# neuromodulation/py_neuromodulation

Hardware: AMD Instinct MI355X
Metric: windows/sec (all features), 256 ch @ 1 kHz (higher is better)
Workload: dtype f32; 1 GPU; 256ch/GPU @1kHz, W=1000, hop=100, 1024 hops/step, all 9 hot-path features, 4 bands, notch50+CAR, z-score normalisation; channels_per_gpu=256, features_per_window=9984, parallelism=channel-shard x1, no collective

## Files before the change

py_neuromodulation_amd/csrc/nmx_engine.inc:

```

#include <algorithm>
#include <chrono>
#include <cmath>
#include <cstdio>
#include <cstdlib>
#include <cstring>
#include <map>
#include <string>
#include <thread>
#include <deque>
#include <functional>
#include <mutex>
#include <condition_variable>
#include <pthread.h>
#include <vector>

#include "../../include/nmx.h"
#include "nmx_k_coh.h"
#include "nmx_k_proj.h"

static thread_local std::string g_nmx_err;
static int nmx_fail(int code, const std::string& msg) {
  g_nmx_err = msg;
  return code;
// ... 44 lines not shown
  NmxFirKernel kernel = NMX_FIR_ONE;
  bool pipelined = false;
  const float* hc = nullptr;
  const float* twc = nullptr;
  bool fused = false;
};
struct FirStage {
  NmxBankArgs a{};
  bool w64 = false;
  NmxBankW64Args w{};
  std::vector<FirLaunch> launches;
  bool takes_dc = true;
};

struct BurstStage {
  NmxHilbertArgs hil{};
  NmxBurstThrArgs bthr{};
  NmxBurstStatArgs bstat{};
  NmxHilbertKind hil_kind = NMX_HIL_FIXED128;
  bool own_hilbert = false;
  bool sparse = false;
  bool sparse_count = false;
  long long env_tail_rows = 0, env_rows = 0;
  NmxBurstStatKind stat_kind = NMX_BSTAT_GENERIC;
  NmxBurstWalk walk{};
  bool fill_split = true;
  int nt_thr = 256;
  long long seen = 0;
  float* d_top = nullptr;
  long long* d_counts = nullptr;
  size_t top_bytes = 0, counts_bytes = 0;
  float* d_floor = nullptr;
  Buf env[2], thr[2];
  Buf env_full[2];
  Buf yb;
  Buf slots;
  int fill_hops(int nw) const { return walk.fill && seen == 0 ? nmx_burst_fill_hops(bthr, nw) : 0; }
};
struct SharpStage {
  NmxSharpArgs a{};
  NmxSharpKind kind = NMX_SHARP_LIST;
  Buf swy[2], todo[2];
  Buf slab;
};
struct KalmanStage {
  NmxKalmanArgs a{};
  double* d_state = nullptr;
  size_t bytes = 0;
};
struct RawNormStage {
  NmxRawNormArgs a{};
  long long hops = 0;
  bool sorted_valid = false;
  size_t ring_bytes = 0, cnt_bytes = 0, len_bytes = 0;
  Buf x_rn, mean, scale;
  Buf qt, qn;
};
// ... 134 lines not shown
```

py_neuromodulation_amd/csrc/nmx_engine_plan_bursts.inc:

```

int build_hilbert(Plan& P) {
  const nmx_plan_desc& d = P.d;
  NmxHilbertArgs& H = P.bursts.hil;
  H.W = d.window;
  H.hil_full = d.window & 1;
  int rc;
  if ((rc = build_fft(P, H.hil_full ? d.window : d.window / 2, &H.hil_r, true))) return rc;
  if ((rc = build_fft(P, d.window, &H.hil_c, true))) return rc;
  H.off_a = 0;
  if (H.hil_full) {
    H.off_b = al4(2 * d.window);
    H.off_y = H.off_b;
    H.lds_floats = H.off_b + al4(2 * d.window);
  } else {
    H.off_b = al4(d.window + 2);
    H.off_y = H.off_b + al4(d.window + 2);
    H.lds_floats = H.off_y + al4(d.window);
  }
  NMX_REQUIRE(H.lds_floats * 4 <= 160 * 1024, "window too long for the Hilbert kernel");
  H.w500_tab = nullptr;
  H.w1000_tab = nullptr;
  if (d.window == 1000) {
    if ((rc = build_w500_tab(P))) return rc;
    H.w500_tab = P.w500_tab;
// ... 6 lines not shown
      t[2 * i + 1] = (float)(scale * std::sin(ang));
    };
    for (int lane = 0; lane < 64; ++lane) {
      const int l = lane < 50 ? lane : 0, k = l % 10;
      for (int r = 1; r < 10; ++r) {
        put((r - 1) * 64 + lane, -2.0 * kPi * ((10 * k * r) % 1000) / 1000.0, 1.0);
        put((8 + r) * 64 + lane, -2.0 * kPi * ((l * r) % 1000) / 1000.0, 1.0);
        put((17 + r) * 64 + lane, -2.0 * kPi * (((l + 50) * r) % 1000) / 1000.0, 1.0);
      }
    }
    for (int k = 0; k < NMX_W1000_CS_N; ++k) put(NMX_W1000_TW_N + k, 2.0 * kPi * k / 2000.0, k ? 2.0 / 2000.0 : 0.0);
    H.w1000_tab = (const float*)upload(P, t.data(), t.size() * sizeof(float));
    if (!H.w1000_tab) return nmx_fail(NMX_E_NOMEM, "table allocation failed");
  }
#endif
  const bool wave = env_int("NMX_HILBERT_W500", 1) != 0;
  P.bursts.hil_kind = wave && d.window == 1000 ? NMX_HIL_W500 : wave && H.w1000_tab ? NMX_HIL_W1000 : NMX_HIL_FIXED128;
  return 0;
}

void burst_floor_reset(Plan& P) {
  const std::vector<float> f((size_t)P.d.n_channels * P.d.n_burst_bands, -INFINITY);
  be_h2d_sync(P.bursts.d_floor, f.data(), f.size() * sizeof(float));
}

static size_t burst_state_bytes(const Plan& P) { return P.bursts.top_bytes + P.bursts.counts_bytes; }
static void burst_state_reset(Plan& P) {
  if (!P.have_bursts) return;
  BurstStage& B = P.bursts;
  be_memset_sync(B.d_top, 0, B.top_bytes);
  be_memset_sync(B.d_counts, 0, B.counts_bytes);
  burst_floor_reset(P);
  B.seen = 0;
}
static void burst_state_export(const Plan& P, char* q) {
  if (!P.have_bursts) return;
  be_d2h_sync(q, P.bursts.d_top, P.bursts.top_bytes);
  be_d2h_sync(q + P.bursts.top_bytes, P.bursts.d_counts, P.bursts.counts_bytes);
}
static int burst_state_import(Plan& P, const char* q, size_t) {
  if (!P.have_bursts) return 0;
  BurstStage& B = P.bursts;
  be_h2d_sync(B.d_top, q, B.top_bytes);
  be_h2d_sync(B.d_counts, q + B.top_bytes, B.counts_bytes);
  memcpy(&B.seen, q + B.top_bytes + sizeof(long long), sizeof(long long));
  burst_floor_reset(P);
// ... 38 lines not shown
  if ((T.K + B.nt_thr - 1) / B.nt_thr > 128) B.nt_thr = 1024;
  NMX_REQUIRE((T.K + B.nt_thr - 1) / B.nt_thr <= (B.nt_thr > 256 ? 64 : 128), "burst top-K list too long for the merge kernel "
              "(sfreq x time_duration_s x (1 - threshold / 100) > 65 536 samples)");
  NMX_REQUIRE(T.lds_floats * 4 <= 160 * 1024,
              "burst threshold state does not fit in 160 KiB LDS (ring x (1 - q) too large)");
  NmxBurstStatArgs& S = B.bstat;
  S.n_outputs = d.n_outputs + d.n_extra_cols;
  S.n_channels = d.n_channels;
  S.n_bands = d.n_burst_bands;
  S.W = d.window;
  S.sfreq = (float)d.sfreq;
  S.seg_s = (float)seg_s;
  S.out_mask = d.burst_out_mask;
  S.cols = cv(d.burst_cols);
  S.off_e = 0;
  S.off_red = al4(d.window + d.window / 16 + 1);
  S.lds_floats = S.off_red + 64;
  const size_t n_state = (size_t)d.n_channels * d.n_burst_bands;
  B.top_bytes = n_state * T.K * sizeof(float);
  B.counts_bytes = n_state * 2 * sizeof(long long);
  B.d_top = (float*)plan_alloc(P, B.top_bytes);
  B.d_counts = (long long*)plan_alloc(P, B.counts_bytes);
  B.d_floor = (float*)plan_alloc(P, n_state * sizeof(float));
  if (!B.d_top || !B.d_counts || !B.d_floor) return nmx_fail(NMX_E_NOMEM, "burst state allocation failed");
  B.own_hilbert = P.bank.w64 || P.bank.a.partitioned;
  B.fill_split = env_int("NMX_FILL_SPLIT", 1) != 0;
  bool wave = env_int("NMX_THR_WAVE", 1) != 0;
#ifdef NMX_HOST_EMU
  wave = false;
#else
  const int sparse = env_int("NMX_BURST_ENV_SPARSE", 1);
  B.sparse = sparse != 0 && B.own_hilbert && (B.hil_kind == NMX_HIL_W500 || B.hil_kind == NMX_HIL_W1000);
  B.sparse_count = sparse == 2;
#endif
  B.walk = nmx_burst_walk_plan(T, env_int("NMX_THR_FILL", 1) != 0, wave, env_int("NMX_THR_LIST_LDS", 1) != 0);
  B.stat_kind = (d.window & 3) || d.window > 2048 ? NMX_BSTAT_GENERIC
                : d.window <= 1024 ? (B.sparse ? NMX_BSTAT_REG16_SPARSE : NMX_BSTAT_REG16)
                                   : (B.sparse ? NMX_BSTAT_REG32_SPARSE : NMX_BSTAT_REG32);
  P.have_bursts = true;
  burst_state_reset(P);
  return 0;
}

static int launch_burst_stage(Plan& P, int par, int nw, float* d_out, be_stream_t s, bool tev) {
  BurstStage& B = P.bursts;
  const int n_seq = P.d.n_channels * P.d.n_burst_bands, W = P.d.window;
  Buf& B_env = B.env[par];
  Buf& B_thr = B.thr[par];
  int rc;
  if ((rc = ensure(B_thr, (size_t)nw * n_seq * sizeof(float)))) return rc;
  be_stream_t sb = s;
  auto fork = [&]() {
    sb = P.stream_b;
    be_event_record(P.ev_fork, s);
    be_stream_wait(sb, P.ev_fork);
  };
  if (P.overlap == 1) fork();
  if (tev) be_timer_start(P.timers[4], sb);
  const unsigned char* env_full = nullptr;
  if (B.own_hilbert) {
    NmxHilbertArgs H = B.hil;
    H.y = (const float*)B.yb.p; H.env = (float*)B_env.p;
    if (B.sparse) {
      if ((rc = ensure(B.env_full[par], (size_t)nw * n_seq))) return rc;
      H.floor = B.d_floor; H.full = (unsigned char*)B.env_full[par].p;
      H.n_seq = n_seq; H.overlap = B.bthr.overlap;
      env_full = H.full;
    }
    be_launch_hilbert(H, B.hil_kind, (long long)nw * n_seq, (size_t)H.lds_floats * 4, sb);
    if (env_full && B.sparse_count) {
      std::vector<unsigned char> f((size_t)nw * n_seq);
      if ((rc = be_sync(sb))) return rc;
      be_d2h_sync(f.data(), env_full, f.size());
      for (unsigned char v : f) B.env_tail_rows += v == 0;
      B.env_rows += (long long)f.size();
    }
  }
  if (P.overlap >= 2) fork();
  NmxBurstThrArgs T = B.bthr;
  T.top = B.d_top; T.counts = B.d_counts; T.floor = B.d_floor;
  NmxBurstWalkSeg seg[3];
  const int n_seg = nmx_burst_walk_schedule(B.walk, T, B.seen, nw, seg);
  for (int i = 0; i < n_seg; ++i) {
    const NmxBurstWalkSeg& g = seg[i];
    T.env = (const float*)B_env.p + (size_t)g.first * n_seq * W;
    T.thr = (float*)B_thr.p + (size_t)g.first * n_seq;
    T.n_windows = g.n;
    if (g.kind == NMX_WALK_FILL) {
      const size_t n_slot = (size_t)n_seq * NMX_FILL_MAX;
      if ((rc = ensure(B.slots, n_slot * (sizeof(unsigned short) + sizeof(float))))) return rc;
      float* sorted = (float*)B.slots.p;
      be_launch_burst_fill(T, n_seq, (unsigned short*)(sorted + n_slot), sorted, B.fill_split, sb);
    } else {
      be_launch_burst_thr(T, B.walk, g, n_seq, B.nt_thr, (size_t)T.lds_floats * 4, sb);
    }
  }
  B.seen += nw;
  NmxBurstStatArgs S = B.bstat;
  S.env = (const float*)B_env.p; S.thr = (const float*)B_thr.p; S.out = d_out; S.n_windows = nw;
  S.full = env_full;
  be_launch_burst_stat(S, B.stat_kind, nw * n_seq, (size_t)S.lds_floats * 4, sb);
  if (tev) be_timer_stop(P.timers[4], sb);
  if (P.overlap) be_event_record(P.ev_join[par], sb);
  return 0;
}
```

py_neuromodulation_amd/csrc/nmx_engine_run.inc:

```
static int run_prep_stages(Plan& P, const float*& src, long long& ch_stride, long long& win_stride,
                           const long long*& starts, int nw, int& clean, be_stream_t s, const NmxBankArgs* fuse_bank = nullptr) {
  const int C = P.d.n_channels, W = P.d.window, Wi = P.w_in;
  int rc;
  auto take = [&](const void* y, int w) {
    src = (const float*)y;
    ch_stride = w; win_stride = (long long)C * w; starts = nullptr; clean = 0;
  };
  for (size_t i = 0; i < P.pre.size(); ++i) {
    Buf& dst = P.x_pf[i & 1];
    if ((rc = ensure(dst, (size_t)nw * C * Wi * sizeof(float)))) return rc;
    NmxBankArgs A = P.pre[i].a;
    A.x = src; A.ch_stride = ch_stride; A.win_stride = win_stride; A.starts = starts; A.clean_on_load = clean;
    A.out = nullptr; A.sw_out = (float*)dst.p;
    launch_fir_stage(P, P.pre[i], A, nw * C, s);
    take(dst.p, Wi);
  }
  if (P.have_notch) {
    if ((rc = ensure(P.y_notch, (size_t)nw * C * Wi * sizeof(float)))) return rc;
    NmxBankArgs A = P.notch.a;
    A.x = src; A.ch_stride = ch_stride; A.win_stride = win_stride; A.starts = starts; A.clean_on_load = clean;
    A.out = nullptr; A.y_out = (float*)P.y_notch.p;
#ifndef NMX_HOST_EMU
    if (fuse_bank) launch_notch_bank_fused(P, A, *fuse_bank, nw * C, s);
    else
// ... 605 lines not shown
    NmxCplx64 *cc = (NmxCplx64*)(d + nx + ny + 2 * nw), *co = cc + L;
    be_launch_rs64_elem(A, NMX_RS64_CHIRP, nullptr, cc, L, 1, s);
    fft(cc, co, L, L, -1, 1);
    A.chirp = cc;
    fft(cur, oth, ld, L, -1, C);
    be_launch_rs64_elem(A, NMX_RS64_MUL, nullptr, cur, L, C, s);
    fft(cur, oth, ld, L, +1, C);
  }
  be_launch_rs64_elem(A, NMX_RS64_OUT, cur, nullptr, final_len, C, s);
  be_d2h_2d_async(y, (size_t)ldy * sizeof(double), d + nx, (size_t)final_len * sizeof(double), (size_t)final_len * sizeof(double),
                  (size_t)C, s);
  rc = be_sync(s);
  be_stream_destroy(s);
  be_free(d);
  return rc ? rc : be_check_launch();
}

int nmx_last_kernels(nmx_plan* plan, int which, char* buf, int64_t n) {
  Plan* P = (Plan*)plan;
  if (!P || !buf || n < 1 || which < 1 || which > 8) return nmx_fail(NMX_E_INVALID, "bad argument");
  std::string k = P->kernels[which];
  if (which == 4 && P->bursts.sparse_count)
    k += (k.empty() ? "" : ",") + std::string("env_tail_rows=") + std::to_string(P->bursts.env_tail_rows) + "/" + std::to_string(P->bursts.env_rows);
  const size_t m = std::min<size_t>(k.size(), (size_t)n - 1);
  memcpy(buf, k.data(), m);
  buf[m] = 0;
  return 0;
}
```

py_neuromodulation_amd/csrc/nmx_k_bank_w64.h:

```cpp
#pragma once

#include "nmx_k_bank.h"
#include "nmx_k_fft500.h"
#include "nmx_k_sharpwave.h"

#ifdef NMX_HOST_EMU
#define NMX_UNROLL
#else
#define NMX_UNROLL _Pragma("unroll")
#endif

#ifdef NMX_HOST_EMU
#define NMX_SCHED_FENCE() ((void)0)
#else
#define NMX_SCHED_FENCE() __builtin_amdgcn_sched_barrier(0)
#endif

#if defined(NMX_BANK_PROFILE) && !defined(NMX_HOST_EMU)
#define NMX_PROF_DECL long long pf_t = clock64(), pf_acc[8] = {0, 0, 0, 0, 0, 0, 0, 0};
#define NMX_PROF(i) { const long long t_ = clock64(); pf_acc[i] += t_ - pf_t; pf_t = t_; }
#define NMX_PROF_PRINT(w, c)                                                                                          \
  if ((w) == 5 && ((c) == 3 || (c) == 40) && (threadIdx.x & 63) == 0)                                                  \
    printf("bank profile w=%d c=%d: load+fwd %lld | spectral+passA %lld | passB load+dft %lld | passB store %lld | "  \
           "passC %lld | variance %lld | series stores %lld | partners %lld (cycles, whole item, %d filters)\n", (w), (c), pf_acc[0],   \
// ... 645 lines not shown
        }
      }
#endif
    }
    NMX_WSYNC();
    NMX_PROF(7)
  }
  NMX_PROF_PRINT(w, c)
}

struct NmxHilbertArgs {
  const float* y;
  float* env;
  int W;
  NmxFft hil_r;
  NmxFft hil_c;
  int hil_full;
  int off_a, off_b, off_y, lds_floats;
  const float* w500_tab;
  const float* w1000_tab;
  const float* floor;
  unsigned char* full;
  int n_seq, overlap;
};

NMX_DEV void nmx_hilbert_item(const NmxHilbertArgs& A, long long item, float* smem) {
  float2* bufA = (float2*)(smem + A.off_a);
  float2* bufB = (float2*)(smem + A.off_b);
  const int W = A.W, Wh = W >> 1;
  const float* src = A.y + item * W;
  float* dst = A.env + item * W;
  if (!A.hil_full) {
    float* ys = smem + A.off_y;
    float* pk = (float*)bufB;
    nmx_stage_row(src, W, [=](int i, float v) { pk[i] = v; ys[i] = v; });
    NMX_SYNC();
    const float2* Zy = nmx_fft_auto<-1, true>(A.hil_r, bufB, bufA, bufB);
    float2* Yb = (Zy == bufA) ? bufB : bufA;
    for (int k = NMX_TID; k <= Wh; k += NMX_NT) Yb[k] = nmx_rfft_bin(Zy, A.hil_r.twr, Wh, k);
    NMX_SYNC();
    float2* Pre = (Yb == bufA) ? bufB : bufA;
    for (int k = NMX_TID; k < Wh; k += NMX_NT) {
      const float2 yk = Yb[k], yn = Yb[Wh - k];
      const float2 xk = k == 0 ? make_float2(0.f, 0.f) : make_float2(yk.y, -yk.x);
      const float2 xn = k == 0 ? make_float2(0.f, 0.f) : make_float2(yn.y, -yn.x);
      Pre[k] = nmx_irfft_pre(xk, xn, A.hil_r.twr[k]);
// ... 18 lines not shown
    else if (k <= (W - 1) / 2) val = make_float2(2.f * Zy[k].x, 2.f * Zy[k].y);
    Ab[k] = make_float2(val.x * invW, val.y * invW);
  }
  NMX_SYNC();
  float2* Zbuf = (Ab == bufA) ? bufB : bufA;
  const float2* an = nmx_fft_auto<+1, true>(A.hil_c, Ab, Zbuf, Ab);
  for (int i = NMX_TID; i < W; i += NMX_NT) dst[i] = nmx_sqrt_fast(an[i].x * an[i].x + an[i].y * an[i].y);
}

#ifndef NMX_HOST_EMU
#define NMX_W500_LDS_FLOATS (1008 + 1000)
template <bool SPARSE>
NMX_DEV void nmx_hilbert_w500_item(const NmxHilbertArgs& A, long long item, float* smem) {
  const int l = NMX_TID;
  nmx_c2* hb = (nmx_c2*)smem;
  nmx_c2* ha = hb + 504;
#ifdef NMX_DEBUG_HILBERT_SAMEROW
  const nmx_rsrc rin = nmx_make_rsrc(A.y + (item & 1023) * 1000, 4000);
#else
  const nmx_rsrc rin = nmx_make_rsrc(A.y + item * 1000, 4000);
#endif
  const nmx_rsrc rout = nmx_make_rsrc(A.env + item * 1000, 4000);
  const float fl = SPARSE ? A.floor[(int)item % A.n_seq] : 0.f;
  NmxW500TwReg T;
  T.load(A.w500_tab, l);
  nmx_c2 y[8];
#pragma unroll
  for (int q = 0; q < 8; ++q) y[q] = __builtin_amdgcn_raw_buffer_load_b64(rin, 8 * l + 512 * q, 0, 0);
#pragma unroll
  for (int q = 0; q < 8; ++q)
    if (q < 7 || l < 52) hb[l + 64 * q] = y[q];
  NMX_WAVE_FENCE();
  const nmx_c2* ht = nmx_w500_hilbert(ha, hb, T, (const nmx_c2*)A.w500_tab + NMX_W500_TW_N, l);
  if (SPARSE) {
    bool hit = !(fl > -INFINITY);
#pragma unroll
    for (int q = 0; q < 8; ++q) {
      const nmx_c2 h = ht[l + 64 * q];
      y[q] = nmx_mk2(nmx_sqrt_fast(y[q].x * y[q].x + h.x * h.x), nmx_sqrt_fast(y[q].y * y[q].y + h.y * h.y));
      hit = hit || ((q < 7 || l < 52) && (y[q].x >= fl || y[q].y >= fl));
    }
    const bool row = __ballot(hit) != 0ull;
    const int keep = 1000 - A.overlap;
#pragma unroll
    for (int q = 0; q < 8; ++q)
      if (row || 2 * (l + 64 * q) + 2 > keep) __builtin_amdgcn_raw_buffer_store_b64(y[q], rout, 8 * l + 512 * q, 0, 0);
    if (l == 0) A.full[item] = row ? 1 : 0;
    return;
  }
#pragma unroll
  for (int q = 0; q < 8; ++q) {
    const nmx_c2 h = ht[l + 64 * q];
    const nmx_c2 e = nmx_mk2(nmx_sqrt_fast(y[q].x * y[q].x + h.x * h.x), nmx_sqrt_fast(y[q].y * y[q].y + h.y * h.y));
    __builtin_amdgcn_raw_buffer_store_b64(e, rout, 8 * l + 512 * q, 0, 0);
  }
}
#define NMX_W1000_LDS_FLOATS 2000
template <bool SPARSE>
NMX_DEV void nmx_hilbert_w1000_item(const NmxHilbertArgs& A, long long item, float* smem) {
  const int l = NMX_TID;
  nmx_c2* hb = (nmx_c2*)smem;
  nmx_c2* ha = hb;
  const nmx_rsrc rin = nmx_make_rsrc(A.y + item * 2000, 8000);
  const nmx_rsrc rout = nmx_make_rsrc(A.env + item * 2000, 8000);
  const float fl = SPARSE ? A.floor[(int)(item % (long long)A.n_seq)] : 0.f;
  NmxW1000TwReg T;
  T.load(A.w1000_tab, l);
  nmx_c2 y[16];
#pragma unroll
  for (int q = 0; q < 16; ++q) y[q] = __builtin_amdgcn_raw_buffer_load_b64(rin, 8 * l + 512 * q, 0, 0);
#pragma unroll
  for (int q = 0; q < 16; ++q)
    if (q < 15 || l < 40) hb[l + 64 * q] = y[q];
  NMX_WAVE_FENCE();
  const nmx_c2* ht = nmx_w1000_hilbert(ha, hb, T, (const nmx_c2*)A.w1000_tab + NMX_W1000_TW_N, l);
  if (SPARSE) {
    bool hit = !(fl > -INFINITY);
#pragma unroll
    for (int q = 0; q < 16; ++q) {
      if (!(q < 15 || l < 40)) continue;
      const nmx_c2 h = ht[l + 64 * q];
      y[q] = nmx_mk2(nmx_sqrt_fast(y[q].x * y[q].x + h.x * h.x), nmx_sqrt_fast(y[q].y * y[q].y + h.y * h.y));
      hit = hit || y[q].x >= fl || y[q].y >= fl;
    }
    const bool row = __ballot(hit) != 0ull;
    const int keep = 2000 - A.overlap;
#pragma unroll
    for (int q = 0; q < 16; ++q)
      if ((q < 15 || l < 40) && (row || 2 * (l + 64 * q) + 2 > keep))
        __builtin_amdgcn_raw_buffer_store_b64(y[q], rout, 8 * l + 512 * q, 0, 0);
    if (l == 0) A.full[item] = row ? 1 : 0;
    return;
  }
#pragma unroll
  for (int q = 0; q < 16; ++q) {
    if (!(q < 15 || l < 40)) continue;
    const nmx_c2 h = ht[l + 64 * q];
    const nmx_c2 e = nmx_mk2(nmx_sqrt_fast(y[q].x * y[q].x + h.x * h.x), nmx_sqrt_fast(y[q].y * y[q].y + h.y * h.y));
    __builtin_amdgcn_raw_buffer_store_b64(e, rout, 8 * l + 512 * q, 0, 0);
  }
}
#endif
```

py_neuromodulation_amd/csrc/nmx_k_bursts.h:

```cpp
#pragma once

#include "nmx_device.h"
#ifdef NMX_HOST_EMU
#include <cstdio>
#include <cstdlib>
#include <vector>
#endif

struct NmxBurstThrArgs {
  const float* env;
  float* thr;
  float* top;
  long long* counts;
  int n_windows, n_channels, n_bands, W;
  int K;
  int n_ring;
  int overlap;
  double q;
  int P2;
  int off_l0, off_l1, off_p, off_red, lds_floats;
  int list_in_global;
  float* floor;
};

NMX_DEV float nmx_burst_floor_of(float v) { return (v - v == 0.f) ? v : -INFINITY; }

NMX_DEV void nmx_bitonic_desc(float* p, int n2) {
  for (int k = 2; k <= n2; k <<= 1) {
    for (int j = k >> 1; j > 0; j >>= 1) {
      for (int i = NMX_TID; i < n2; i += NMX_NT) {
        const int ixj = i ^ j;
        if (ixj > i) {
          const float a = p[i], b = p[ixj];
          const bool desc = ((i & k) == 0);
          if (desc ? (a < b) : (a > b)) {
            p[i] = b;
            p[ixj] = a;
          }
        }
      }
      NMX_SYNC();
    }
  }
}

// ... 126 lines not shown
#else
  float vals[CH];
#endif
  const bool steady_ok = A.P2 >= NMX_THR_P && K > 2 * NMX_THR_F && A.overlap <= 256;
  bool steady = false;
  int Lm = 0, nF = 0, nP = 0;
  const long long m_ring = A.n_ring;
  const double pos_ring = A.q * (double)(m_ring - 1);
  const long long lo_ring = (long long)floor(pos_ring);
  const double frac_ring = pos_ring - (double)lo_ring;
  const int ia_ring = (int)(m_ring - 1 - lo_ring);

  const bool can_prefetch = A.overlap <= NMX_NT;
  float pre = 0.f;
  bool have_pre = false;
  NMX_SYNC();
  for (int w = 0; w < A.n_windows; ++w) {
    const int n_new = (nwin == 0) ? W : A.overlap;
    const int n4 = (n_new + 3) & ~3;
    const float* e = A.env + (((long long)w * A.n_channels + c) * A.n_bands + bi) * W + (W - n_new);
    if (have_pre) {
      if (NMX_TID < n_new) pc[NMX_TID] = pre;
    } else {
      for (int i = NMX_TID; i < n_new; i += NMX_NT) pc[i] = e[i];
    }
    for (int i = n_new + NMX_TID; i < n4; i += NMX_NT) pc[i] = -INFINITY;
    have_pre = false;
    if (can_prefetch && w + 1 < A.n_windows) {
      const float* en = A.env + (((long long)(w + 1) * A.n_channels + c) * A.n_bands + bi) * W + (W - A.overlap);
      if (NMX_TID < A.overlap) pre = en[NMX_TID];
      have_pre = true;
    }
    const bool want_steady = steady_ok && total >= m_ring && len == K && ia_ring >= K - 3 && ia_ring < K;
    if (want_steady && !steady) {
      nF = NMX_THR_FREFILL;
      Lm = K - nF;
      nP = 0;
      NMX_SYNC();
      for (int j = NMX_TID; j < nF; j += NMX_NT) F[j] = L[K - 1 - j];
      steady = true;
#ifdef NMX_HOST_EMU
      if (getenv("NMX_EMU_TRACE")) fprintf(stderr, "[emu] steady regime entered at hop %d (c=%d b=%d)\n", w, c, bi);
#endif
    }
    if (NMX_TID == 0) { cnts[0] = 0; cnts[1] = 0; cnts[2] = 0; }
    NMX_SYNC();
    if (!steady) {
      nmx_rank_sort_desc(pc, n_new, ps);
      NMX_SYNC();
      len = nmx_merge_into<CH>(L, len, K, ps, ins, n_new, vals);
      total += n_new;
      nwin += 1;
      if (NMX_TID == 0) {
// ... 52 lines not shown
      NMX_SYNC();
      for (int i = NMX_TID; i < nP; i += NMX_NT) pc[i] = Pp[i];
      for (int i = nP + NMX_TID; i < ((nP + 3) & ~3); i += NMX_NT) pc[i] = -INFINITY;
      NMX_SYNC();
      nmx_rank_sort_desc(pc, nP, ps);
      NMX_SYNC();
      Lm = nmx_merge_into<CH>(L, Lm, K, ps, ins, nP, vals);
      for (int j = NMX_TID; j < nF; j += NMX_NT) L[Lm + j] = F[nF - 1 - j];
      NMX_SYNC();
      nF = NMX_THR_FREFILL;
      Lm = K - nF;
      nP = 0;
      for (int j = NMX_TID; j < nF; j += NMX_NT) F[j] = L[K - 1 - j];
      NMX_SYNC();
    }
  }
  NMX_SYNC();
  if (!A.list_in_global) for (int i = NMX_TID; i < len; i += NMX_NT) gtop[i] = L[i];
  if (NMX_TID == 0) {
    A.counts[2 * sidx] = total;
    A.counts[2 * sidx + 1] = nwin;
    if (A.floor && A.n_windows > 0)
      A.floor[sidx] = (total >= m_ring && ia_ring >= 0 && ia_ring < len) ? nmx_burst_floor_of(L[ia_ring]) : -INFINITY;
  }
}

#define NMX_THRW_PF 16
#define NMX_THRW_I 256
#define NMX_THRW_PF_LL 8
#define NMX_THRW_PF_OF(NR, LL) ((NR) == 2 ? ((LL) ? NMX_THRW_PF_LL : NMX_THRW_PF) : 4)
#define NMX_THRW_LDS_FLOATS_OF(NR, LL) (2 * 256 * (NR) + 3 * ((NR) == 2 ? NMX_THR_P : 512) + NMX_THRW_I + NMX_THRW_PF_OF(NR, LL) * 64 * (NR))
#define NMX_THRW_LDS_FLOATS_NR(NR) NMX_THRW_LDS_FLOATS_OF(NR, false)
#define NMX_THRW_LDS_FLOATS NMX_THRW_LDS_FLOATS_NR(2)

#define NMX_WALK_NEVER 0x7fffffffffffffffLL
static inline int nmx_burst_thrw_nr(const NmxBurstThrArgs& A) { return A.overlap <= 128 ? 2 : 4; }
static inline long long nmx_burst_wave_from(const NmxBurstThrArgs& A) {
  const int nr = nmx_burst_thrw_nr(A);
  if (A.overlap < 1 || A.overlap > 256 || A.overlap + 8 >= 192 * nr) return NMX_WALK_NEVER;
  const long long m_ring = A.n_ring;
  const long long lo_ring = (long long)floor(A.q * (double)(m_ring - 1));
  const int ia_ring = (int)(m_ring - 1 - lo_ring);
  if (!(A.K > 2 * 256 * nr && ia_ring >= A.K - 3 && ia_ring < A.K)) return NMX_WALK_NEVER;
  const long long short_of = m_ring - A.W;
  return short_of <= 0 ? 1 : 1 + (short_of + A.overlap - 1) / A.overlap;
}
// ... 103 lines not shown
#pragma unroll
      for (int q = 0; q < 8; ++q) { const int j = j0 + 64 * q + lane; t8[q] = j < K ? Lg[j] : 0.f; }
#pragma unroll
      for (int q = 0; q < 8; ++q) { const int j = j0 + 64 * q + lane; if (j < K) L[j] = t8[q]; }
    }
    NMX_WAVE_FENCE();
  }
  long long total = A.counts[2 * sidx];
  long long nwin = A.counts[2 * sidx + 1];
  const long long m_ring = A.n_ring;
  const double pos_ring = A.q * (double)(m_ring - 1);
  const long long lo_ring = (long long)floor(pos_ring);
  const double frac_ring = pos_ring - (double)lo_ring;
  const int ja = K - 1 - (int)(m_ring - 1 - lo_ring);

  int nF = TREFILL, fh = 0, Lm = K - nF, nP = 0;
  for (int j = lane; j < nF; j += 64) F[j] = L[K - 1 - j];
  NMX_WAVE_FENCE();
  float T = F[0], Fmax = F[nF - 1];
  float thr_cur = nmx_lerp_thr((double)F[ja], (double)F[ja + 1], frac_ring, true);

  const long long hop_stride = (long long)A.n_channels * A.n_bands * W;
  const float* e0 = A.env + ((long long)c * A.n_bands + bi) * W + (W - ov);
  float nx[NR][PF];
#pragma unroll
  for (int u = 0; u < PF; ++u) {
    const float* e = e0 + (long long)u * hop_stride;
    const bool in = u < A.n_windows;
#pragma unroll
    for (int q = 0; q < NR; ++q) nx[q][u] = (in && lane + 64 * q < ov) ? e[lane + 64 * q] : -INFINITY;
  }
  for (int w0 = 0; w0 < A.n_windows; w0 += PF) {
#pragma unroll
    for (int u = 0; u < PF; ++u) {
#pragma unroll
      for (int q = 0; q < NR; ++q) stage[64 * NR * u + 64 * q + lane] = nx[q][u];
    }
#pragma unroll
    for (int u = 0; u < PF; ++u) {
      const int w = w0 + PF + u;
      const float* e = e0 + (long long)w * hop_stride;
      const bool in = w < A.n_windows;
#pragma unroll
      for (int q = 0; q < NR; ++q) nx[q][u] = (in && lane + 64 * q < ov) ? e[lane + 64 * q] : -INFINITY;
    }
    NMX_WAVE_FENCE();
    NMX_TP(0)
    const int ng = (A.n_windows - w0) < PF ? (A.n_windows - w0) : PF;
#pragma nounroll
    for (int u = 0; u < ng; ++u) {
      const int w = w0 + u;
      float x[NR];
      bool cc[NR];
      unsigned long long bm[NR];
      int a = 0;
#pragma unroll
      for (int q = 0; q < NR; ++q) {
        x[q] = stage[64 * NR * u + 64 * q + lane];
        cc[q] = x[q] > T;
        bm[q] = __ballot(cc[q]);
        a += __popcll(bm[q]);
      }
      NMX_TP(1)
      if (a) {
        const unsigned long long below = (1ull << lane) - 1ull;
        bool ii[NR];
        unsigned long long bim[NR];
        int nI = 0, np_new = 0;
#pragma unroll
        for (int q = 0; q < NR; ++q) {
          ii[q] = cc[q] && x[q] <= Fmax;
// ... 195 lines not shown
        NMX_WAVE_FENCE();
        T = F[0];
        Fmax = F[nF - 1];
#ifdef NMX_THRW_PROFILE
        ++n_flush;
#endif
        NMX_TP(6)
      }
    }
  }
#ifdef NMX_THRW_PROFILE
  if (lane == 0 && (sidx == 0 || sidx == 311))
    printf("[thrw %lld] hops %d inserts %d flushes %d | cycles: top %lld classify %lld fringe %lld store %lld sort %lld stream %lld recut %lld\n",
           sidx, A.n_windows, n_ins, n_flush, tp[0], tp[1], tp[2], tp[3], tp[4], tp[5], tp[6]);
#endif
  if (LL) {
    NMX_WAVE_FENCE();
    for (int j = lane; j < K; j += 64) Lg[j] = L[j];
  }
  if (lane == 0) {
    A.counts[2 * sidx] = total;
    A.counts[2 * sidx + 1] = nwin;
    if (A.floor && A.n_windows > 0) A.floor[sidx] = nmx_burst_floor_of(F[fh + ja]);
  }
}
#endif

struct NmxBurstStatArgs {
  const float* env;
  const float* thr;
  float* out;
  int n_outputs, n_windows, n_channels, n_bands, W;
  float sfreq, seg_s;
  unsigned out_mask;
  NmxCols cols;
  int off_e, off_red, lds_floats;
  const unsigned char* full;
};

NMX_DEV void nmx_burst_stat_zero(const NmxBurstStatArgs& A, int w, int c, int bi) {
  float* row = A.out + (long long)w * A.n_outputs;
  int col = A.cols.base + c * A.cols.ch_stride + bi * A.cols.a_stride;
  for (int s = 0; s < 6; ++s)
    if (A.out_mask & (1u << s)) {
      row[col] = 0.f;
      col += A.cols.b_stride;
    }
}

#ifdef NMX_HOST_EMU
NMX_DEV double nmx_wave_excl_sum_d(double v, double* total) { *total = v; return 0.0; }
NMX_DEV void nmx_wave_excl_latest(int& pos, double& val) { pos = -1; val = 0.0; }
#else
NMX_DEV double nmx_dpp_d(double v, double ident, int ctrl_sel) {
  const long long vb = __builtin_bit_cast(long long, v), ib = __builtin_bit_cast(long long, ident);
  int lo = (int)(vb & 0xffffffffll), hi = (int)(vb >> 32);
  const int ilo = (int)(ib & 0xffffffffll), ihi = (int)(ib >> 32);
  switch (ctrl_sel) {
    case 0: lo = __builtin_amdgcn_update_dpp(ilo, lo, 0x111, 0xf, 0xf, false); hi = __builtin_amdgcn_update_dpp(ihi, hi, 0x111, 0xf, 0xf, false); break;
    case 1: lo = __builtin_amdgcn_update_dpp(ilo, lo, 0x112, 0xf, 0xf, false); hi = __builtin_amdgcn_update_dpp(ihi, hi, 0x112, 0xf, 0xf, false); break;
// ... 129 lines not shown
```

py_neuromodulation_amd/csrc/nmx_wave.hip:

```cpp
#ifndef NMX_NT_FIXED
#error "compile with -DNMX_NT_FIXED=64"
#endif
#include <hip/hip_runtime.h>
#include <cstdio>
#include <cstdlib>

#include <cstdlib>

#include "nmx_k_bursts.h"
#include "nmx_k_bank_w64.h"
#include "nmx_k_burst_stat_reg.h"
#include "nmx_k_scan.h"
#include "nmx_k_td.h"
#include "nmx_k_timeosc_w1000.h"
#include "nmx_k_timeosc_w510.h"
#include "nmx_k_sharpwave.h"

extern __shared__ __attribute__((aligned(16))) float nmx_smem_wave[];

static int waves_per_wg(size_t lds_one, int dflt = 1) {
  const char* v = getenv("NMX_WAVES_PER_WG");
  const int k = (v && atoi(v) >= 1 && atoi(v) <= 4) ? atoi(v) : 0;
  int kk = k ? k : dflt;
  while (kk > 1 && lds_one * kk > 64 * 1024) --kk;
  return kk;
}
#define NMX_WAVE_ITEM(item, smem, n_items, slice)                                                   \
  const int wave_ = __builtin_amdgcn_readfirstlane((int)(threadIdx.x >> 6));                        \
  const int item = (int)blockIdx.x * (int)(blockDim.x >> 6) + wave_;                                \
  if (item >= (n_items)) return;                                                                    \
  float* smem = nmx_smem_wave + wave_ * (slice)

__global__ void __launch_bounds__(256) nmx_kern_burst_stat(const NmxBurstStatArgs A, int n_items, int slice) {
  const int wave = __builtin_amdgcn_readfirstlane((int)(threadIdx.x >> 6));
  const int item = blockIdx.x * (blockDim.x >> 6) + wave;
  if (item >= n_items) return;
  const int bi = item % A.n_bands, r = item / A.n_bands;
  nmx_burst_stat_item(A, r / A.n_channels, r % A.n_channels, bi, nmx_smem_wave + wave * slice);
}

template <int CH, bool SPARSE = false>
__global__ void __launch_bounds__(256) nmx_kern_burst_stat_reg(const NmxBurstStatArgs A, int n_items) {
  const int wave = __builtin_amdgcn_readfirstlane((int)(threadIdx.x >> 6));
  const int item = blockIdx.x * 4 + wave;
  if (item >= n_items) return;
  const int bi = item % A.n_bands, r = item / A.n_bands;
  nmx_burst_stat_item_reg<CH, SPARSE>(A, r / A.n_channels, r % A.n_channels, bi);
}

__global__ void __launch_bounds__(256) nmx_kern_sharp(const NmxSharpArgs A, int n_items, int slice) {
  const int wave = __builtin_amdgcn_readfirstlane((int)(threadIdx.x >> 6));
  const int item = blockIdx.x * (blockDim.x >> 6) + wave;
  if (item >= n_items) return;
  const int fi = item % A.n_filters, r = item / A.n_filters;
  nmx_sharp_item(A, r / A.n_channels, r % A.n_channels, fi, nmx_smem_wave + wave * slice);
}

template <int NR, bool LL>
__global__ void __launch_bounds__(64) nmx_kern_burst_thr_wave(const NmxBurstThrArgs A) {
  __builtin_amdgcn_s_setprio(3);
  const int item = blockIdx.x;
  nmx_burst_thr_wave_item<NR, LL>(A, item / A.n_bands, item % A.n_bands, nmx_smem_wave);
}

extern "C" void nmx_wave_launch_burst_thr(const NmxBurstThrArgs* A, int n_items, int nr, bool list_lds, size_t lds, hipStream_t s) {
  static unsigned long long seen = 0;
// ... 287 lines not shown
      NMX_SYNC();
    }
  }
}

extern "C" void nmx_wave_launch_sharp_todo(const NmxSharpArgs* A, int n_items, size_t lds, const unsigned char* todo,
                                           hipStream_t s) {
  static unsigned long long seen = 0;
  if (nmx_first_on_device(seen)) {
    (void)hipFuncSetAttribute((const void*)nmx_kern_sharp_todo, hipFuncAttributeMaxDynamicSharedMemorySize, 160 * 1024);
  }
  const int blocks = (n_items + 63) / 64;
  const int grid = blocks < 256 * 14 ? blocks : 256 * 14;
  hipLaunchKernelGGL(nmx_kern_sharp_todo, dim3(grid), dim3(64), lds, s, *A, n_items, todo);
  nmxi_note_kernel("nmx_kern_sharp_todo");
}

extern "C" void nmx_wave_launch_burst_stat(const NmxBurstStatArgs* A, NmxBurstStatKind kind, int n_items, size_t lds, hipStream_t s) {
  static unsigned long long seen = 0;
  if (nmx_first_on_device(seen)) {
    (void)hipFuncSetAttribute((const void*)nmx_kern_burst_stat, hipFuncAttributeMaxDynamicSharedMemorySize, 160 * 1024);
  }
  const dim3 grid4((n_items + 3) / 4);
  switch (kind) {
    case NMX_BSTAT_REG16_SPARSE: hipLaunchKernelGGL((nmx_kern_burst_stat_reg<16, true>), grid4, dim3(256), 0, s, *A, n_items); nmxi_note_kernel("nmx_kern_burst_stat_reg_sparse<16>"); return;
    case NMX_BSTAT_REG16: hipLaunchKernelGGL(nmx_kern_burst_stat_reg<16>, grid4, dim3(256), 0, s, *A, n_items); nmxi_note_kernel("nmx_kern_burst_stat_reg<16>"); return;
    case NMX_BSTAT_REG32_SPARSE: hipLaunchKernelGGL((nmx_kern_burst_stat_reg<32, true>), grid4, dim3(256), 0, s, *A, n_items); nmxi_note_kernel("nmx_kern_burst_stat_reg_sparse<32>"); return;
    case NMX_BSTAT_REG32: hipLaunchKernelGGL(nmx_kern_burst_stat_reg<32>, grid4, dim3(256), 0, s, *A, n_items); nmxi_note_kernel("nmx_kern_burst_stat_reg<32>"); return;
    case NMX_BSTAT_GENERIC: break;
  }
  const int k = waves_per_wg(lds);
  const int slice = (int)((lds / 4 + 3) & ~(size_t)3);
  hipLaunchKernelGGL(nmx_kern_burst_stat, dim3((n_items + k - 1) / k), dim3(64 * k), (size_t)slice * 4 * k, s, *A,
                     n_items, slice);
  nmxi_note_kernel("nmx_kern_burst_stat");
}

extern "C" void nmx_wave_launch_sharp(const NmxSharpArgs* A, int n_items, size_t lds, hipStream_t s) {
  static unsigned long long seen = 0;
  if (nmx_first_on_device(seen)) {
    (void)hipFuncSetAttribute((const void*)nmx_kern_sharp, hipFuncAttributeMaxDynamicSharedMemorySize, 160 * 1024);
  }
  const int k = waves_per_wg(lds, 2);
  const int slice = (int)((lds / 4 + 3) & ~(size_t)3);
  hipLaunchKernelGGL(nmx_kern_sharp, dim3((n_items + k - 1) / k), dim3(64 * k), (size_t)slice * 4 * k, s, *A,
                     n_items, slice);
  nmxi_note_kernel("nmx_kern_sharp");
}
```

Baseline: 165,800 windows/s.

## Skip burst threshold walk for hops whose new envelope tail cannot enter the top list

The Hilbert kernel now tracks a per-sequence keep_min (smallest retained top-list value). It writes a per-hop walk flag only when a new tail sample exceeds it, and skips storing tail envelope samples otherwise. The threshold walk kernels read these flags and treat unflagged hops as -inf, fast-forwarding quiet groups of windows. Burst stat gains a rows-per-wave sparse variant that zero-fills non-full rows and loops only over flagged items. This cuts memory traffic and walk work at the cost of extra flag state and more complex control flow.

Result: no change. 167,300 windows/s, median of 6 (+0.9%).

```diff
diff --git a/py_neuromodulation_amd/csrc/nmx_engine.inc b/py_neuromodulation_amd/csrc/nmx_engine.inc
--- a/py_neuromodulation_amd/csrc/nmx_engine.inc
+++ b/py_neuromodulation_amd/csrc/nmx_engine.inc
@@ -90,6 +90,8 @@
   bool sparse = false;
   bool sparse_count = false;
   long long env_tail_rows = 0, env_rows = 0;
+  int walk_sparse = 0;
+  long long walk_hops = 0, walk_hops_of = 0;
   NmxBurstStatKind stat_kind = NMX_BSTAT_GENERIC;
   NmxBurstWalk walk{};
   bool fill_split = true;
@@ -99,8 +101,10 @@
   long long* d_counts = nullptr;
   size_t top_bytes = 0, counts_bytes = 0;
   float* d_floor = nullptr;
+  float* d_keep_min = nullptr;
   Buf env[2], thr[2];
   Buf env_full[2];
+  Buf env_walk[2];
   Buf yb;
   Buf slots;
   int fill_hops(int nw) const { return walk.fill && seen == 0 ? nmx_burst_fill_hops(bthr, nw) : 0; }
diff --git a/py_neuromodulation_amd/csrc/nmx_engine_plan_bursts.inc b/py_neuromodulation_amd/csrc/nmx_engine_plan_bursts.inc
--- a/py_neuromodulation_amd/csrc/nmx_engine_plan_bursts.inc
+++ b/py_neuromodulation_amd/csrc/nmx_engine_plan_bursts.inc
@@ -52,6 +52,7 @@
 void burst_floor_reset(Plan& P) {
   const std::vector<float> f((size_t)P.d.n_channels * P.d.n_burst_bands, -INFINITY);
   be_h2d_sync(P.bursts.d_floor, f.data(), f.size() * sizeof(float));
+  be_h2d_sync(P.bursts.d_keep_min, f.data(), f.size() * sizeof(float));
 }
 
 static size_t burst_state_bytes(const Plan& P) { return P.bursts.top_bytes + P.bursts.counts_bytes; }
@@ -136,7 +137,8 @@
   B.d_top = (float*)plan_alloc(P, B.top_bytes);
   B.d_counts = (long long*)plan_alloc(P, B.counts_bytes);
   B.d_floor = (float*)plan_alloc(P, n_state * sizeof(float));
-  if (!B.d_top || !B.d_counts || !B.d_floor) return nmx_fail(NMX_E_NOMEM, "burst state allocation failed");
+  B.d_keep_min = (float*)plan_alloc(P, n_state * sizeof(float));
+  if (!B.d_top || !B.d_counts || !B.d_floor || !B.d_keep_min) return nmx_fail(NMX_E_NOMEM, "burst state allocation failed");
   B.own_hilbert = P.bank.w64 || P.bank.a.partitioned;
   B.fill_split = env_int("NMX_FILL_SPLIT", 1) != 0;
   bool wave = env_int("NMX_THR_WAVE", 1) != 0;
@@ -146,6 +148,11 @@
   const int sparse = env_int("NMX_BURST_ENV_SPARSE", 1);
   B.sparse = sparse != 0 && B.own_hilbert && (B.hil_kind == NMX_HIL_W500 || B.hil_kind == NMX_HIL_W1000);
   B.sparse_count = sparse == 2;
+  B.walk_sparse = B.sparse ? env_int("NMX_BURST_WALK_SPARSE", 1) : 0;
+  NMX_REQUIRE(B.walk_sparse >= 0 && B.walk_sparse <= 2, "NMX_BURST_WALK_SPARSE must be 0, 1 or 2");
+  B.bstat.rows_per_wave = B.walk_sparse ? env_int("NMX_BURST_STAT_ROWS", 16) : 0;
+  NMX_REQUIRE(B.bstat.rows_per_wave == 0 || B.bstat.rows_per_wave == 16 || B.bstat.rows_per_wave == 64,
+              "NMX_BURST_STAT_ROWS must be 0, 16 or 64");
 #endif
   B.walk = nmx_burst_walk_plan(T, env_int("NMX_THR_FILL", 1) != 0, wave, env_int("NMX_THR_LIST_LDS", 1) != 0);
   B.stat_kind = (d.window & 3) || d.window > 2048 ? NMX_BSTAT_GENERIC
@@ -171,7 +178,7 @@
   };
   if (P.overlap == 1) fork();
   if (tev) be_timer_start(P.timers[4], sb);
-  const unsigned char* env_full = nullptr;
+  const unsigned char *env_full = nullptr, *env_walk = nullptr;
   if (B.own_hilbert) {
     NmxHilbertArgs H = B.hil;
     H.y = (const float*)B.yb.p; H.env = (float*)B_env.p;
@@ -180,6 +187,11 @@
       H.floor = B.d_floor; H.full = (unsigned char*)B.env_full[par].p;
       H.n_seq = n_seq; H.overlap = B.bthr.overlap;
       env_full = H.full;
+      if (B.walk_sparse) {
+        if ((rc = ensure(B.env_walk[par], (size_t)nw * n_seq))) return rc;
+        H.keep_min = B.d_keep_min; H.walk = (unsigned char*)B.env_walk[par].p;
+        env_walk = H.walk;
+      }
     }
     be_launch_hilbert(H, B.hil_kind, (long long)nw * n_seq, (size_t)H.lds_floats * 4, sb);
     if (env_full && B.sparse_count) {
@@ -189,16 +201,24 @@
       for (unsigned char v : f) B.env_tail_rows += v == 0;
       B.env_rows += (long long)f.size();
     }
+    if (env_walk && B.walk_sparse == 2) {
+      std::vector<unsigned char> f((size_t)nw * n_seq);
+      if ((rc = be_sync(sb))) return rc;
+      be_d2h_sync(f.data(), env_walk, f.size());
+      for (unsigned char v : f) B.walk_hops += v != 0;
+      B.walk_hops_of += (long long)f.size();
+    }
   }
   if (P.overlap >= 2) fork();
   NmxBurstThrArgs T = B.bthr;
-  T.top = B.d_top; T.counts = B.d_counts; T.floor = B.d_floor;
+  T.top = B.d_top; T.counts = B.d_counts; T.floor = B.d_floor; T.keep_min = B.d_keep_min;
   NmxBurstWalkSeg seg[3];
   const int n_seg = nmx_burst_walk_schedule(B.walk, T, B.seen, nw, seg);
   for (int i = 0; i < n_seg; ++i) {
     const NmxBurstWalkSeg& g = seg[i];
     T.env = (const float*)B_env.p + (size_t)g.first * n_seq * W;
     T.thr = (float*)B_thr.p + (size_t)g.first * n_seq;
+    T.walk = env_walk && g.kind != NMX_WALK_FILL ? env_walk + (size_t)g.first * n_seq : nullptr;
     T.n_windows = g.n;
     if (g.kind == NMX_WALK_FILL) {
       const size_t n_slot = (size_t)n_seq * NMX_FILL_MAX;
diff --git a/py_neuromodulation_amd/csrc/nmx_engine_run.inc b/py_neuromodulation_amd/csrc/nmx_engine_run.inc
--- a/py_neuromodulation_amd/csrc/nmx_engine_run.inc
+++ b/py_neuromodulation_amd/csrc/nmx_engine_run.inc
@@ -651,6 +651,8 @@
   std::string k = P->kernels[which];
   if (which == 4 && P->bursts.sparse_count)
     k += (k.empty() ? "" : ",") + std::string("env_tail_rows=") + std::to_string(P->bursts.env_tail_rows) + "/" + std::to_string(P->bursts.env_rows);
+  if (which == 4 && P->bursts.walk_sparse == 2)
+    k += (k.empty() ? "" : ",") + std::string("walk_hops=") + std::to_string(P->bursts.walk_hops) + "/" + std::to_string(P->bursts.walk_hops_of);
   const size_t m = std::min<size_t>(k.size(), (size_t)n - 1);
   memcpy(buf, k.data(), m);
   buf[m] = 0;
diff --git a/py_neuromodulation_amd/csrc/nmx_k_bank_w64.h b/py_neuromodulation_amd/csrc/nmx_k_bank_w64.h
--- a/py_neuromodulation_amd/csrc/nmx_k_bank_w64.h
+++ b/py_neuromodulation_amd/csrc/nmx_k_bank_w64.h
@@ -691,6 +691,8 @@
   const float* floor;
   unsigned char* full;
   int n_seq, overlap;
+  const float* keep_min;
+  unsigned char* walk;
 };
 
 NMX_DEV void nmx_hilbert_item(const NmxHilbertArgs& A, long long item, float* smem) {
@@ -755,6 +757,7 @@
 #endif
   const nmx_rsrc rout = nmx_make_rsrc(A.env + item * 1000, 4000);
   const float fl = SPARSE ? A.floor[(int)item % A.n_seq] : 0.f;
+  const float km = (SPARSE && A.walk) ? A.keep_min[(int)item % A.n_seq] : 0.f;
   NmxW500TwReg T;
   T.load(A.w500_tab, l);
   nmx_c2 y[8];
@@ -767,18 +770,28 @@
   const nmx_c2* ht = nmx_w500_hilbert(ha, hb, T, (const nmx_c2*)A.w500_tab + NMX_W500_TW_N, l);
   if (SPARSE) {
     bool hit = !(fl > -INFINITY);
+    bool wk = false;
+    const int keep = 1000 - A.overlap;
 #pragma unroll
     for (int q = 0; q < 8; ++q) {
       const nmx_c2 h = ht[l + 64 * q];
       y[q] = nmx_mk2(nmx_sqrt_fast(y[q].x * y[q].x + h.x * h.x), nmx_sqrt_fast(y[q].y * y[q].y + h.y * h.y));
       hit = hit || ((q < 7 || l < 52) && (y[q].x >= fl || y[q].y >= fl));
     }
+#pragma unroll
+    for (int q = 0; q < 8; ++q) {
+      const int i0 = 2 * (l + 64 * q);
+      wk |= (q < 7 || l < 52) & (((i0 >= keep) & !(y[q].x <= km)) | ((i0 + 1 >= keep) & !(y[q].y <= km)));
+    }
     const bool row = __ballot(hit) != 0ull;
-    const int keep = 1000 - A.overlap;
+    const bool tail = !A.walk || __ballot(wk) != 0ull;
 #pragma unroll
     for (int q = 0; q < 8; ++q)
-      if (row || 2 * (l + 64 * q) + 2 > keep) __builtin_amdgcn_raw_buffer_store_b64(y[q], rout, 8 * l + 512 * q, 0, 0);
-    if (l == 0) A.full[item] = row ? 1 : 0;
+      if (row || (tail && 2 * (l + 64 * q) + 2 > keep)) __builtin_amdgcn_raw_buffer_store_b64(y[q], rout, 8 * l + 512 * q, 0, 0);
+    if (l == 0) {
+      A.full[item] = row ? 1 : 0;
+      if (A.walk) A.walk[item] = tail ? 1 : 0;
+    }
     return;
   }
 #pragma unroll
@@ -797,6 +810,7 @@
   const nmx_rsrc rin = nmx_make_rsrc(A.y + item * 2000, 8000);
   const nmx_rsrc rout = nmx_make_rsrc(A.env + item * 2000, 8000);
   const float fl = SPARSE ? A.floor[(int)(item % (long long)A.n_seq)] : 0.f;
+  const float km = (SPARSE && A.walk) ? A.keep_min[(int)(item % (long long)A.n_seq)] : 0.f;
   NmxW1000TwReg T;
   T.load(A.w1000_tab, l);
   nmx_c2 y[16];
@@ -809,6 +823,8 @@
   const nmx_c2* ht = nmx_w1000_hilbert(ha, hb, T, (const nmx_c2*)A.w1000_tab + NMX_W1000_TW_N, l);
   if (SPARSE) {
     bool hit = !(fl > -INFINITY);
+    bool wk = false;
+    const int keep = 2000 - A.overlap;
 #pragma unroll
     for (int q = 0; q < 16; ++q) {
       if (!(q < 15 || l < 40)) continue;
@@ -816,13 +832,21 @@
       y[q] = nmx_mk2(nmx_sqrt_fast(y[q].x * y[q].x + h.x * h.x), nmx_sqrt_fast(y[q].y * y[q].y + h.y * h.y));
       hit = hit || y[q].x >= fl || y[q].y >= fl;
     }
+#pragma unroll
+    for (int q = 0; q < 16; ++q) {
+      const int i0 = 2 * (l + 64 * q);
+      wk |= (q < 15 || l < 40) & (((i0 >= keep) & !(y[q].x <= km)) | ((i0 + 1 >= keep) & !(y[q].y <= km)));
+    }
     const bool row = __ballot(hit) != 0ull;
-    const int keep = 2000 - A.overlap;
+    const bool tail = !A.walk || __ballot(wk) != 0ull;
 #pragma unroll
     for (int q = 0; q < 16; ++q)
-      if ((q < 15 || l < 40) && (row || 2 * (l + 64 * q) + 2 > keep))
+      if ((q < 15 || l < 40) && (row || (tail && 2 * (l + 64 * q) + 2 > keep)))
         __builtin_amdgcn_raw_buffer_store_b64(y[q], rout, 8 * l + 512 * q, 0, 0);
-    if (l == 0) A.full[item] = row ? 1 : 0;
+    if (l == 0) {
+      A.full[item] = row ? 1 : 0;
+      if (A.walk) A.walk[item] = tail ? 1 : 0;
+    }
     return;
   }
 #pragma unroll
diff --git a/py_neuromodulation_amd/csrc/nmx_k_bursts.h b/py_neuromodulation_amd/csrc/nmx_k_bursts.h
--- a/py_neuromodulation_amd/csrc/nmx_k_bursts.h
+++ b/py_neuromodulation_amd/csrc/nmx_k_bursts.h
@@ -21,6 +21,8 @@
   int off_l0, off_l1, off_p, off_red, lds_floats;
   int list_in_global;
   float* floor;
+  float* keep_min;
+  const unsigned char* walk;
 };
 
 NMX_DEV float nmx_burst_floor_of(float v) { return (v - v == 0.f) ? v : -INFINITY; }
@@ -193,13 +195,16 @@
     if (have_pre) {
       if (NMX_TID < n_new) pc[NMX_TID] = pre;
     } else {
-      for (int i = NMX_TID; i < n_new; i += NMX_NT) pc[i] = e[i];
+      const bool flagged = !A.walk || A.walk[((long long)w * A.n_channels + c) * A.n_bands + bi] != 0;
+      for (int i = NMX_TID; i < n_new; i += NMX_NT) pc[i] = flagged ? e[i] : -INFINITY;
     }
     for (int i = n_new + NMX_TID; i < n4; i += NMX_NT) pc[i] = -INFINITY;
     have_pre = false;
     if (can_prefetch && w + 1 < A.n_windows) {
-      const float* en = A.env + (((long long)(w + 1) * A.n_channels + c) * A.n_bands + bi) * W + (W - A.overlap);
-      if (NMX_TID < A.overlap) pre = en[NMX_TID];
+      const long long in = ((long long)(w + 1) * A.n_channels + c) * A.n_bands + bi;
+      const float* en = A.env + in * W + (W - A.overlap);
+      const bool flagged = !A.walk || A.walk[in] != 0;
+      if (NMX_TID < A.overlap) pre = flagged ? en[NMX_TID] : -INFINITY;
       have_pre = true;
     }
     const bool want_steady = steady_ok && total >= m_ring && len == K && ia_ring >= K - 3 && ia_ring < K;
@@ -298,6 +303,8 @@
     A.counts[2 * sidx + 1] = nwin;
     if (A.floor && A.n_windows > 0)
       A.floor[sidx] = (total >= m_ring && ia_ring >= 0 && ia_ring < len) ? nmx_burst_floor_of(L[ia_ring]) : -INFINITY;
+    if (A.keep_min && A.n_windows > 0)
+      A.keep_min[sidx] = (total >= m_ring && len == K) ? nmx_burst_floor_of(L[K - 1]) : -INFINITY;
   }
 }
 
@@ -447,31 +454,48 @@
 
   const long long hop_stride = (long long)A.n_channels * A.n_bands * W;
   const float* e0 = A.env + ((long long)c * A.n_bands + bi) * W + (W - ov);
+  const long long seq_stride = (long long)A.n_channels * A.n_bands;
+  const unsigned char* wf0 = A.walk ? A.walk + sidx : nullptr;
+  auto flag_of = [&](int w) -> int { return (wf0 && lane < PF && w < A.n_windows) ? (int)wf0[(long long)w * seq_stride] : (wf0 ? 0 : 1); };
+  unsigned long long fm_cur = __ballot(flag_of(lane) != 0);
+  int fb_next = flag_of(PF + lane);
   float nx[NR][PF];
 #pragma unroll
   for (int u = 0; u < PF; ++u) {
     const float* e = e0 + (long long)u * hop_stride;
-    const bool in = u < A.n_windows;
+    const bool in = u < A.n_windows && ((fm_cur >> u) & 1ull);
 #pragma unroll
     for (int q = 0; q < NR; ++q) nx[q][u] = (in && lane + 64 * q < ov) ? e[lane + 64 * q] : -INFINITY;
   }
   for (int w0 = 0; w0 < A.n_windows; w0 += PF) {
-#pragma unroll
-    for (int u = 0; u < PF; ++u) {
-#pragma unroll
-      for (int q = 0; q < NR; ++q) stage[64 * NR * u + 64 * q + lane] = nx[q][u];
+    const int ng = (A.n_windows - w0) < PF ? (A.n_windows - w0) : PF;
+    const unsigned long long fm_next = __ballot(fb_next != 0);
+    fb_next = flag_of(w0 + 2 * PF + lane);
+    const bool quiet = fm_cur == 0ull && w0 + ng < A.n_windows;
+    if (!quiet) {
+#pragma unroll
+      for (int u = 0; u < PF; ++u) {
+#pragma unroll
+        for (int q = 0; q < NR; ++q) stage[64 * NR * u + 64 * q + lane] = nx[q][u];
+      }
     }
 #pragma unroll
     for (int u = 0; u < PF; ++u) {
       const int w = w0 + PF + u;
       const float* e = e0 + (long long)w * hop_stride;
-      const bool in = w < A.n_windows;
+      const bool in = w < A.n_windows && ((fm_next >> u) & 1ull);
 #pragma unroll
       for (int q = 0; q < NR; ++q) nx[q][u] = (in && lane + 64 * q < ov) ? e[lane + 64 * q] : -INFINITY;
+    }
+    fm_cur = fm_next;
+    if (quiet) {
+      if (lane < ng) A.thr[(long long)(w0 + lane) * seq_stride + sidx] = thr_cur;
+      total += (long long)ng * ov;
+      nwin += ng;
+      continue;
     }
     NMX_WAVE_FENCE();
     NMX_TP(0)
-    const int ng = (A.n_windows - w0) < PF ? (A.n_windows - w0) : PF;
 #pragma nounroll
     for (int u = 0; u < ng; ++u) {
       const int w = w0 + u;
@@ -713,6 +737,7 @@
     A.counts[2 * sidx] = total;
     A.counts[2 * sidx + 1] = nwin;
     if (A.floor && A.n_windows > 0) A.floor[sidx] = nmx_burst_floor_of(F[fh + ja]);
+    if (A.keep_min && A.n_windows > 0) A.keep_min[sidx] = nmx_burst_floor_of(F[fh]);
   }
 }
 #endif
@@ -727,6 +752,7 @@
   NmxCols cols;
   int off_e, off_red, lds_floats;
   const unsigned char* full;
+  int rows_per_wave;
 };
 
 NMX_DEV void nmx_burst_stat_zero(const NmxBurstStatArgs& A, int w, int c, int bi) {
diff --git a/py_neuromodulation_amd/csrc/nmx_wave.hip b/py_neuromodulation_amd/csrc/nmx_wave.hip
--- a/py_neuromodulation_amd/csrc/nmx_wave.hip
+++ b/py_neuromodulation_amd/csrc/nmx_wave.hip
@@ -39,9 +39,29 @@
   nmx_burst_stat_item(A, r / A.n_channels, r % A.n_channels, bi, nmx_smem_wave + wave * slice);
 }
 
-template <int CH, bool SPARSE = false>
+template <int CH, bool SPARSE = false, int RW = 0>
 __global__ void __launch_bounds__(256) nmx_kern_burst_stat_reg(const NmxBurstStatArgs A, int n_items) {
   const int wave = __builtin_amdgcn_readfirstlane((int)(threadIdx.x >> 6));
+  if (SPARSE && RW > 0) {
+    const int lane = (int)(threadIdx.x & 63);
+    const int base = ((int)blockIdx.x * 4 + wave) * RW;
+    if (base >= n_items) return;
+    const int mine = base + lane;
+    const bool in = lane < RW && mine < n_items;
+    const bool whole = in && A.full[mine] != 0;
+    if (in && !whole) {
+      const int r = mine / A.n_bands;
+      nmx_burst_stat_zero(A, r / A.n_channels, r % A.n_channels, mine % A.n_bands);
+    }
+    unsigned long long m = __ballot(whole);
+    while (m) {
+      const int item = __builtin_amdgcn_readfirstlane(base + (int)__ffsll((long long)m) - 1);
+      m &= m - 1;
+      const int bi = item % A.n_bands, r = item / A.n_bands;
+      nmx_burst_stat_item_reg<CH, false>(A, r / A.n_channels, r % A.n_channels, bi);
+    }
+    return;
+  }
   const int item = blockIdx.x * 4 + wave;
   if (item >= n_items) return;
   const int bi = item % A.n_bands, r = item / A.n_bands;
@@ -375,10 +395,22 @@
     (void)hipFuncSetAttribute((const void*)nmx_kern_burst_stat, hipFuncAttributeMaxDynamicSharedMemorySize, 160 * 1024);
   }
   const dim3 grid4((n_items + 3) / 4);
+  const int rw = n_items >= 131072 ? A->rows_per_wave : 0;
+  const dim3 gridw((unsigned)((n_items + 4 * (rw ? rw : 1) - 1) / (4 * (rw ? rw : 1))));
   switch (kind) {
-    case NMX_BSTAT_REG16_SPARSE: hipLaunchKernelGGL((nmx_kern_burst_stat_reg<16, true>), grid4, dim3(256), 0, s, *A, n_items); nmxi_note_kernel("nmx_kern_burst_stat_reg_sparse<16>"); return;
+    case NMX_BSTAT_REG16_SPARSE:
+      if (rw == 64) hipLaunchKernelGGL((nmx_kern_burst_stat_reg<16, true, 64>), gridw, dim3(256), 0, s, *A, n_items);
+      else if (rw == 16) hipLaunchKernelGGL((nmx_kern_burst_stat_reg<16, true, 16>), gridw, dim3(256), 0, s, *A, n_items);
+      else hipLaunchKernelGGL((nmx_kern_burst_stat_reg<16, true>), grid4, dim3(256), 0, s, *A, n_items);
+      nmxi_note_kernel("nmx_kern_burst_stat_reg_sparse<16>");
+      return;
     case NMX_BSTAT_REG16: hipLaunchKernelGGL(nmx_kern_burst_stat_reg<16>, grid4, dim3(256), 0, s, *A, n_items); nmxi_note_kernel("nmx_kern_burst_stat_reg<16>"); return;
-    case NMX_BSTAT_REG32_SPARSE: hipLaunchKernelGGL((nmx_kern_burst_stat_reg<32, true>), grid4, dim3(256), 0, s, *A, n_items); nmxi_note_kernel("nmx_kern_burst_stat_reg_sparse<32>"); return;
+    case NMX_BSTAT_REG32_SPARSE:
+      if (rw == 64) hipLaunchKernelGGL((nmx_kern_burst_stat_reg<32, true, 64>), gridw, dim3(256), 0, s, *A, n_items);
+      else if (rw == 16) hipLaunchKernelGGL((nmx_kern_burst_stat_reg<32, true, 16>), gridw, dim3(256), 0, s, *A, n_items);
+      else hipLaunchKernelGGL((nmx_kern_burst_stat_reg<32, true>), grid4, dim3(256), 0, s, *A, n_items);
+      nmxi_note_kernel("nmx_kern_burst_stat_reg_sparse<32>");
+      return;
     case NMX_BSTAT_REG32: hipLaunchKernelGGL(nmx_kern_burst_stat_reg<32>, grid4, dim3(256), 0, s, *A, n_items); nmxi_note_kernel("nmx_kern_burst_stat_reg<32>"); return;
     case NMX_BSTAT_GENERIC: break;
   }
```
